# crowsonkb/style_transfer

Hardware: AMD Instinct MI355X
Metric: tile-iterations/sec, VGG-19 2048px/1024-tile (fwd+bwd, Gram/content losses, regularizers, Adam step) (higher is better)
Workload: dtype f32 (fp16x2-split MFMA, fp32 accumulate)

## Files before the change

### include/stx.h

```cpp
#ifndef STX_H_
#define STX_H_

#include <stddef.h>
#include <stdint.h>

#ifdef __cplusplus
extern "C" {
#endif

typedef struct stx_engine stx_engine;

typedef enum stx_status {
    STX_OK = 0,
    STX_ERR_ARG = -1,
    STX_ERR_HIP = -2,
    STX_ERR_STATE = -3,
    STX_ERR_UNSUPPORTED = -4,
    STX_ERR_NOMEM = -5
} stx_status;

typedef enum stx_mem { STX_HOST = 0, STX_DEVICE = 1 } stx_mem;

typedef enum stx_layer_type {
    STX_LAYER_INPUT = 0, STX_LAYER_CONV = 1, STX_LAYER_RELU = 2, STX_LAYER_POOL = 3
// ... 14 lines not shown
} stx_layer_desc;

const char *stx_version(void);
const char *stx_last_error(void);
int stx_reread_env(void);
int stx_device_count(int *count);
int stx_device_name(int device, char *buf, size_t buf_len);

int stx_engine_create(int device, const stx_layer_desc *layers, int n_layers, stx_engine **out);
int stx_engine_create_shared(stx_engine *primary, stx_engine **out);
void stx_engine_destroy(stx_engine *e);
int stx_set_conv_weights(stx_engine *e, const char *conv_layer, const float *weights,
                         const float *bias, int mem);
int stx_sync(stx_engine *e);
int stx_fence(stx_engine *e, unsigned long long *ticket);
int stx_fence_wait(stx_engine *e, unsigned long long ticket);
int stx_engine_wait(stx_engine *e, stx_engine *other);
typedef enum stx_query {
    STX_Q_SHARED_ENGINES = 0,
    STX_Q_TARGET_UPLOADS = 1,
    STX_Q_TARGET_BYTES = 2,
    STX_Q_WEIGHT_BYTES = 3,
    STX_Q_TILE_EVALS = 4,
    STX_Q_PEERS_WITHOUT_ACCESS = 5
} stx_query;
int stx_engine_query(stx_engine *e, int what, double *value);
int stx_engine_device(stx_engine *e, int *device);
int stx_engine_stream(stx_engine *e, void **hip_stream);

int stx_malloc(stx_engine *e, size_t bytes, void **dev_ptr);
int stx_free(stx_engine *e, void *dev_ptr);
int stx_memset_async(stx_engine *e, void *dev_ptr, int value, size_t bytes);
int stx_memcpy_async(stx_engine *e, void *dst, int dst_mem, const void *src, int src_mem,
                     size_t bytes);

typedef struct stx_content_target {
    int content_index;
    const char *layer;
    int channels, height, width;
    const float *features;
    int mem;
} stx_content_target;

typedef struct stx_style_target {
    int style_index;
    const char *layer;
    int channels;
// ... 232 lines not shown
```

### style_transfer_amd/build.py

```python

import concurrent.futures
import os
import subprocess
import sys

CSRC = os.path.join(os.path.dirname(os.path.abspath(__file__)), 'csrc')
REPO = os.path.dirname(os.path.dirname(os.path.abspath(__file__)))
INCLUDE = os.path.join(REPO, 'include')
LIB = os.path.join(CSRC, 'libstx.so')
HIPCC = os.environ.get('HIPCC', '/opt/rocm/bin/hipcc')
ARCH = 'gfx950'

SOURCES = {
    'conv_mfma.hip': [],
    'conv_wino2.hip': [],
    'conv_first.hip': [],
    'conv_h2.hip': [],
    'gram.hip': [],
    'symm.hip': [],
    'pool.hip': [],
    'reduce.hip': [],
    'content_mask.hip': [],
    'image_ops.hip': ['-ffp-contract=off'],
    'swt.hip': ['-ffp-contract=off'],
    'style_mask.hip': ['-ffp-contract=off'],
    'lap.hip': ['-ffp-contract=off'],
    'stat.hip': ['-ffp-contract=off'],
    'photo.hip': ['-ffp-contract=off'],
    'nnfm.hip': ['-ffp-contract=off'],
    'conv_dispatch.cpp': [],
    'engine.cpp': [],
    'targets.cpp': [],
    'tile_path.cpp': [],
    'tile_terms.cpp': [],
    'image_api.cpp': [],
    'op_hooks.cpp': [],
}
EXTRA = os.environ.get('STX_HIPCC_EXTRA', '').split()
COMMON = EXTRA + ['--offload-arch=' + ARCH, '-O3', '-std=c++17', '-fPIC', '-I' + INCLUDE, '-I' + CSRC,
          '-Wall', '-Wno-unused-function']


def _stale(target, deps):
    if not os.path.exists(target):
        return True
    t = os.path.getmtime(target)
    return any(os.path.getmtime(d) > t for d in deps)


def _compile(src, extra, force):
    obj = os.path.join(CSRC, os.path.splitext(src)[0] + '.o')
    path = os.path.join(CSRC, src)
    deps = [path, os.path.join(CSRC, 'common.h'), os.path.join(CSRC, 'bf16x3.h'),
            os.path.join(CSRC, 'f16x2.h'), os.path.join(CSRC, 'engine.h'), os.path.join(INCLUDE, 'stx.h')]
    if force or _stale(obj, deps):
        cmd = [HIPCC] + COMMON + extra + ['-c', path, '-o', obj]
        proc = subprocess.run(cmd, stdout=subprocess.PIPE, stderr=subprocess.STDOUT, text=True)
        if proc.returncode != 0:
            raise RuntimeError('hipcc failed on %s:\n%s' % (src, proc.stdout))
        if proc.stdout.strip():
            sys.stderr.write(proc.stdout)
    return obj


def build(force=False, verbose=False):
    with concurrent.futures.ThreadPoolExecutor(max_workers=min(16, len(SOURCES))) as ex:
        futs = [ex.submit(_compile, src, extra, force) for src, extra in SOURCES.items()]
        objs = [f.result() for f in futs]
    if force or _stale(LIB, objs):
        cmd = [HIPCC, '--offload-arch=' + ARCH, '-shared', '-fPIC', '-o', LIB] + objs
        proc = subprocess.run(cmd, stdout=subprocess.PIPE, stderr=subprocess.STDOUT, text=True)
        if proc.returncode != 0:
            raise RuntimeError('link failed:\n' + proc.stdout)
    if verbose:
        print('built', LIB)
    return LIB

# ... 4 lines not shown
```

### style_transfer_amd/csrc/common.h

```cpp
#pragma once

#include <hip/hip_runtime.h>

#include <vector>

#include <cstdarg>
#include <cstdio>
#include <functional>
#include <string>

#include "stx.h"

namespace stx {

constexpr float kEps = 1.1920928955078125e-07f;

void set_error(const char *fmt, ...);

const char *sw_env(const char *name);
void sw_reread();

#define STX_HIP(call)                                                                       \
    do {                                                                                    \
        hipError_t err__ = (call);                                                          \
// ... 98 lines not shown
    const float *mask;
    float *partials;
    int K, M, H, W;
    int ksize;
    int relu;
    int epilogue;
    ConvInject inject;
    unsigned char *pool_codes = nullptr;
    unsigned char *in_codes = nullptr;
    const unsigned char *mask_codes = nullptr;
    unsigned char *out_codes = nullptr;
    bool wants_codes = false;
    bool skip_y = false;
    float *pool_out = nullptr;
    int pool_mode = 0;
    float *splitk_ws = nullptr;
    size_t splitk_ws_floats = 0;
    long long *clock_out = nullptr;
    const unsigned *x_amax = nullptr;
    unsigned *y_amax = nullptr;
    const unsigned char *pin_codes = nullptr;
    int pin_mode = 0;
    bool pin_mask = false;
#ifdef STX_EXPERIMENT_BF3
    const void *x_split = nullptr;
#endif
};

enum class ConvFamily { Direct, Wino2, H2 };

struct ConvConfig {
    ConvFamily family;
    int id;
    int bm;
    int kc;
    int pr, pc;
    int threads;
    size_t lds_bytes;
};

ConvConfig conv_pick_config(int ksize, int K, int M, int H, int W);
ConvConfig conv_config_by_id(int id);
bool direct_takes_inject(const ConvConfig &cfg);
int conv_num_workgroups(const ConvConfig &cfg, int M, int H, int W);
size_t conv_packed_floats(const ConvConfig &cfg, int K, int M, int ksize);
int conv_pack_weights(hipStream_t s, const float *w_caffe, int Mo, int Ko, int ksize,
// ... 50 lines not shown
                      int K, int H, int W, int relu, float *gram_partials, unsigned *y_amax = nullptr);

ConvConfig wino2_config(int geometry = 0);
int wino2_pick_geometry(int H, int W);
size_t wino2_packed_floats(int K, int M);
int wino2_pack_weights(hipStream_t s, const float *w_caffe, int Mo, int Ko, int transpose_flip,
                       float *packed);
int wino2_launch(hipStream_t s, const ConvConfig &cfg, const ConvProblem &p, int ksplit);
bool wino2_fuses_pool(const ConvProblem &p);
bool wino2_uses_relu_codes(const ConvProblem &p, int ksplit);
bool wino2_writes_out_codes(const ConvConfig &cfg, const ConvProblem &p);
int wino2_splitk_factor(const ConvConfig &cfg, const ConvProblem &p);
struct Wino2Tail { int items, slices; };
Wino2Tail wino2_tail_split(const ConvConfig &cfg, const ConvProblem &p);
int wino2_max_slices(const ConvConfig &cfg, const ConvProblem &p);

constexpr int kAmaxSlots = 64;
ConvConfig h2_config(int mb, int pb = 1);
ConvConfig h2_pick_config(const ConvProblem &p);
bool h2_usable(const ConvProblem &p);
size_t h2_packed_floats(int K, int M);
int h2_pack_weights(hipStream_t s, const float *w_caffe, int Mo, int Ko, int transpose_flip, float *packed);
int h2_launch(hipStream_t s, const ConvConfig &cfg, const ConvProblem &p, int ksplit);
int h2_splitk_factor(const ConvConfig &cfg, const ConvProblem &p);
bool h2_fuses_pool(const ConvProblem &p);
bool h2_takes_pooled_input(const ConvConfig &cfg, const ConvProblem &p);
int absmax_launch(hipStream_t s, const float *x, size_t n, unsigned *slots);

size_t conv_small_packed_floats(int K);
int conv_small_pack(hipStream_t s, const float *w_caffe, int Mo, int Ko, int transpose_flip,
                    float *packed);
int conv_small_launch(hipStream_t s, const float *x, const float *packed, float *y,
                      const float *mask, int K, int M, int H, int W);

bool conv_h2_enabled();
struct ConvTuner { int device; hipStream_t stream; hipEvent_t ev0, ev1; std::function<int(const ConvConfig &, const float **)> bank; };
int conv_choose(const ConvProblem &p, bool winograd, const ConvTuner *tuner, ConvConfig *out);
struct ConvBank { int key; size_t floats; std::function<int(hipStream_t, const float *w_caffe, float *packed)> pack; };
ConvBank conv_bank(const ConvConfig &cfg, int dir, int Mo, int Ko, int ksize);
ConvBank conv_small_bank(int Mo, int Ko);
int conv_dispatch(hipStream_t s, const ConvConfig &cfg, const ConvProblem &p, double *flop_algorithmic,
                  double *flop_issued);
int conv_splitk_factor(const ConvConfig &cfg, const ConvProblem &p);
size_t conv_splitk_floats(const ConvConfig &cfg, const ConvProblem &p);
bool conv_takes_clock(const ConvConfig &cfg);
bool conv_fuses_pool(const ConvConfig &cfg, const ConvProblem &p);
// ... 220 lines not shown
```

### style_transfer_amd/csrc/conv_h2.hip

```cpp

#include <algorithm>
#include <cstdlib>
#include <type_traits>

#include "common.h"
#include "f16x2.h"

#ifndef STX_H2_SKIP
#define STX_H2_SKIP 0
#endif

namespace stx {

namespace {

typedef _Float16 f16x8 __attribute__((ext_vector_type(8)));
typedef float f32x16 __attribute__((ext_vector_type(16)));
typedef float f32x4 __attribute__((ext_vector_type(4)));
typedef float f32x2 __attribute__((ext_vector_type(2)));
typedef unsigned int u32x4 __attribute__((ext_vector_type(4)));
typedef unsigned int u32x3 __attribute__((ext_vector_type(3)));
typedef unsigned int u32x2v __attribute__((__vector_size__(2 * sizeof(unsigned int))));

constexpr int KC = 16;
// ... 21 lines not shown
template <int I, int N, typename F>
__device__ __forceinline__ void static_for(F &&f) {
    if constexpr (I < N) {
        f(std::integral_constant<int, I>{});
        static_for<I + 1, N>(f);
    }
}

__device__ __forceinline__ void lds_barrier() {
    asm volatile("s_waitcnt lgkmcnt(0)\n\ts_barrier" ::: "memory");
}


}

#ifdef STX_H2_TIMING
__device__ long long g_h2_timing[8][8];
__device__ long long g_h2_epi[8][8];
#define STX_H2_STAMP(i) if (pass == 0) t_epi[i] = clock64()
#else
#define STX_H2_STAMP(i)
#endif

template <int EPI, int MB, int PB, int PIN>
__global__ __launch_bounds__(NT) void conv_h2_kernel(WinoArgs a) {
    using G = Geo<PB>;
    [[maybe_unused]] constexpr int PR = G::PR, RT = G::RT, V_PIECE = G::V_PIECE, V_BYTES = G::V_BYTES, NU = G::NU, FULL = G::FULL;
    constexpr size_t kLdsBytes = G::kLds;
    constexpr int NJ = 4 * PB;
    extern __shared__ __attribute__((aligned(16))) char ldsb[];
#ifdef STX_H2_TIMING
    const long long t_start = clock64(), w_start = wall_clock64();
#endif
    constexpr int BM = 64 * MB;

    const int tid = threadIdx.x, lane = tid & 63;
    const int wave = sgpr(tid >> 6);
    const int xi = wave & 3, wh = wave >> 2;
    const int l31 = lane & 31, half = lane >> 5;

    const int m_tiles = a.m_tiles, a_tiles_x = a.tiles_x, a_tiles_y = a.tiles_y, a_H = a.H, a_W = a.W;
    const int a_n_chunks = a.n_chunks, a_ksplit = a.ksplit, a_item_base = a.item_base, a_x_bytes = a.x_bytes,
              a_w_bytes = a.w_bytes;
    const float *const a_x = a.x, *const a_w = a.w;
    asm volatile("" ::"s"(m_tiles), "s"(a_tiles_x), "s"(a_tiles_y), "s"(a_H), "s"(a_W), "s"(a_n_chunks), "s"(a_ksplit),
                 "s"(a_item_base), "s"(a_x_bytes), "s"(a_w_bytes), "s"(a_x), "s"(a_w));
    const int nb = gridDim.x, xcd = blockIdx.x & 7, slot_x = blockIdx.x >> 3;
    const int q8 = nb >> 3, r8 = nb & 7;
// ... 253 lines not shown
#pragma unroll
        for (int q = 0; q < 2; ++q) bq[slot][q] = *reinterpret_cast<const f16x8 *>(vb + q * V_PIECE);
    };

#ifdef STX_H2_TIMING
    const long long t_p0 = clock64();
#endif
    static_for<0, NU>([&](auto n_c) __attribute__((always_inline)) { x_load(decltype(n_c)::value, c_begin); });
    if (LEAN) {
        a_load(0, 0, c_begin);
    } else {
#pragma unroll
        for (int ky = 0; ky < 3; ++ky) a_load(ky, ky, c_begin);
    }
    __builtin_amdgcn_sched_barrier(0);
    read_scales();
#pragma unroll
    for (int b = 0; b < MB; ++b)
#pragma unroll
        for (int j = 0; j < NJ; ++j) asm volatile("" : "+v"(acc[b][j]));
    float s_scale = 0.f, c_scale = 0.f;
    if (EPI == kEpiDgradInject) {
        const float n = (float)((size_t)a.M * HW);
        if (a.inj.sgrad) s_scale = a.inj.s_coef * (1.0f / (a.inj.s_abs_sum[0] / n + kEps));
        if (a.inj.content) c_scale = a.inj.c_coef * (1.0f / (a.inj.c_sums[1] / n + kEps));
    }
    const int hh = wave & 1, mrow = (wave >> 1) & 1, rqp = wave >> 2;
    const bool weven = (a.W & 1) == 0;
    const int xx0 = x0 + 2 * (l31 & 15);
    const unsigned plane_bytes = (unsigned)a.M * HW4;
    const __amdgpu_buffer_rsrc_t ry = __builtin_amdgcn_make_buffer_rsrc(
        a.y + (EPI == kEpiPartial ? (size_t)kslice * a.M * HW : 0), 0, (int)plane_bytes, 0x00020000);
    const __amdgpu_buffer_rsrc_t rmask = __builtin_amdgcn_make_buffer_rsrc(
        const_cast<float *>(a.mask), 0, a.mask ? (int)plane_bytes : 0, 0x00020000);
    const __amdgpu_buffer_rsrc_t rsg = __builtin_amdgcn_make_buffer_rsrc(
        const_cast<float *>(a.inj.sgrad), 0, a.inj.sgrad ? (int)plane_bytes : 0, 0x00020000);
    const __amdgpu_buffer_rsrc_t rft = __builtin_amdgcn_make_buffer_rsrc(
        const_cast<float *>(a.inj.feat), 0, a.inj.feat ? (int)plane_bytes : 0, 0x00020000);
    const __amdgpu_buffer_rsrc_t rbias = __builtin_amdgcn_make_buffer_rsrc(
        const_cast<float *>(a.bias), 0, a.bias ? a.M * 4 : 0, 0x00020000);
    const int ph = (a.H + 1) >> 1, pw = (a.W + 1) >> 1;
    const __amdgpu_buffer_rsrc_t rpool = __builtin_amdgcn_make_buffer_rsrc(
        a.pool_out, 0, a.pool_out ? a.M * ph * pw * 4 : 0, 0x00020000);
    const __amdgpu_buffer_rsrc_t rcodes = __builtin_amdgcn_make_buffer_rsrc(
        a.pool_codes, 0, a.pool_codes ? a.M * ph * pw : 0, 0x00020000);
    const int cph = (a.H + 1) >> 1, cpw = (a.W + 1) >> 1;
    const __amdgpu_buffer_rsrc_t rmc = __builtin_amdgcn_make_buffer_rsrc(
        const_cast<unsigned char *>(a.mask_codes), 0, a.mask_codes ? a.M * cph * cpw : 0, 0x00020000);
// ... 29 lines not shown
        if (decltype(even_c)::value)
            return __builtin_bit_cast(f32x2, __builtin_amdgcn_raw_buffer_load_b64(rs, lr.vo[y][0], so, 0));
        f32x2 v;
        v.x = __builtin_bit_cast(float, __builtin_amdgcn_raw_buffer_load_b32(rs, lr.vo[y][0], so, 0));
        v.y = __builtin_bit_cast(float, __builtin_amdgcn_raw_buffer_load_b32(rs, lr.vo[y][1], so, 0));
        return v;
    };
    auto st2 = [&](const __amdgpu_buffer_rsrc_t &rs, const LaneRows &lr, int y, unsigned so, f32x2 v, auto even_c)
                   __attribute__((always_inline)) {
        if (STX_H2_SKIP & 8) {
            if (v.x == 1.2345e-30f) __builtin_amdgcn_raw_buffer_store_b32(0u, rs, lr.vo[y][0], so, 0);
            return;
        }
        if (decltype(even_c)::value) {
            __builtin_amdgcn_raw_buffer_store_b64(__builtin_bit_cast(u32x2v, v), rs, lr.vo[y][0], so, 0);
        } else {
            const float v0 = v.x, v1 = v.y;
            __builtin_amdgcn_raw_buffer_store_b32(__builtin_bit_cast(unsigned, v0), rs, lr.vo[y][0], so, 0);
            __builtin_amdgcn_raw_buffer_store_b32(__builtin_bit_cast(unsigned, v1), rs, lr.vo[y][1], so, 0);
        }
    };
    int ccol[2] = {0, 0};
    auto content_columns = [&](const LaneRows &lr) __attribute__((always_inline)) {
        if (EPI == kEpiDgradInject && content) {
#pragma unroll
            for (int e = 0; e < 2; ++e) {
                const bool ok = lr.yy < a.H && xx0 < a.W;
                const int x = ok ? (xx0 + e < a.W ? xx0 + e : xx0) : (e && 1 < a.W ? 1 : 0);
                int r = (cw_ox + x) % cw_cw;
                ccol[e] = r < 0 ? r + cw_cw : r;
            }
        }
    };
    if (HOIST) content_columns(rows0);
#ifdef STX_H2_TIMING
    __builtin_amdgcn_sched_barrier(0);
    const long long t_p1 = clock64();
    asm volatile("s_waitcnt vmcnt(0)" ::: "memory");
    const long long t_p2 = clock64();
#endif
    static_for<0, NU>([&](auto n_c) __attribute__((always_inline)) {
        constexpr int n = decltype(n_c)::value;
        stage_all(n, 0);
        if (c_begin + 1 < c_end) x_load(n, c_begin + 1);
    });
#ifdef STX_H2_TIMING
    __builtin_amdgcn_sched_barrier(0);
// ... 83 lines not shown
    if (mark) {
        const long long dc = clock64() - mark_c, dw = wall_clock64() - mark_w;
        if (tid == 0) {
            a.clock_out[0] = dw >= 100 ? dc : 0;
            a.clock_out[1] = dw >= 100 ? dw : 0;
        }
    }
#ifdef STX_H2_TIMING
    const long long t_end = clock64(), w_end = wall_clock64();
#endif

    float amax = 0.f;
    f32x4 *ex = reinterpret_cast<f32x4 *>(ldsb);

#ifdef STX_H2_TIMING
    long long t_epi[4] = {0, 0, 0, 0};
#endif
    auto epilogue_pass = [&](auto pass_c, auto even_c) __attribute__((always_inline)) {
        constexpr int pass = decltype(pass_c)::value;
        constexpr int mbi = pass % MB, pbi = pass / MB;
        const LaneRows lr = pbi == 0 && HOIST ? rows0 : lane_rows(pbi);
        if (!HOIST && pass == 0) content_columns(lr);
        int crow[2] = {0, 0};
        if (EPI == kEpiDgradInject && content) {
#pragma unroll
            for (int y = 0; y < 2; ++y) {
                const bool ok = lr.yy + y < a.H && xx0 < a.W;
                int q = (cw_oy + (ok ? lr.yy + y : 0)) % cw_ch;
                crow[y] = (q < 0 ? q + cw_ch : q) * cw_cw;
            }
        }
        const int cblk = m0 + (hh * MB + mbi) * 32;
        auto chan = [&](int n) __attribute__((always_inline)) {
            const int c0 = cblk + (n & 3) + 8 * (2 * rqp + (n >> 2));
            return sgpr(c0 < M_ ? c0 : M_);
        };
        float bs[8];
        f32x2 mk[16], sg[16];
        unsigned mkb[8];
#pragma unroll
        for (int n = 0; n < 8; ++n) {
            const int c = chan(n);
            const unsigned so = (unsigned)c * HW4;
            if (EPI == kEpiForward) {
                bs[n] = a.bias ? __builtin_bit_cast(float, __builtin_amdgcn_raw_buffer_load_b32(
                                                               rbias, (unsigned)half * 16u, (unsigned)c * 4u, 0))
                               : 0.f;
            } else if (EPI != kEpiPartial) {
                if (a.mask_codes) mkb[n] = __builtin_amdgcn_raw_buffer_load_b8(rmc, lr.vmc, (unsigned)(c * cph * cpw), 0);
#pragma unroll
                for (int y = 0; y < 2; ++y) {
                    if (!a.mask_codes && a.mask && !(STX_H2_SKIP & 16)) mk[2 * n + y] = ld2(rmask, lr, y, so, even_c);
                    if (EPI == kEpiDgradInject && a.inj.sgrad) sg[2 * n + y] = ld2(rsg, lr, y, so, even_c);
                }
            }
        }
        STX_H2_STAMP(0);
        __syncthreads();
        STX_H2_STAMP(1);
#pragma unroll
        for (int j = 0; j < 4; ++j)
#pragma unroll
            for (int rq = 0; rq < 4; ++rq)
                ex[(((xi * 2 + wh) * 4 + j) * 4 + rq) * 64 + lane] =
                    f32x4{acc[mbi][4 * pbi + j][4 * rq], acc[mbi][4 * pbi + j][4 * rq + 1],
                          acc[mbi][4 * pbi + j][4 * rq + 2], acc[mbi][4 * pbi + j][4 * rq + 3]};
        __syncthreads();
        STX_H2_STAMP(2);
#pragma unroll
        for (int rqi = 0; rqi < 2; ++rqi) {
            const int rq = 2 * rqp + rqi;
            f32x4 o[2][2];
#pragma unroll
            for (int s = 0; s < 2; ++s) {
                f32x4 p[4];
#pragma unroll
// ... 1 lines not shown
                o[s][0] = (p[0] + p[1] + p[2]) * out_scale * out_scale2;
                o[s][1] = (p[1] - p[2] - p[3]) * out_scale * out_scale2;
            }
#pragma unroll
            for (int e = 0; e < 4; ++e) {
                const int n = 4 * rqi + e;
                const int c = chan(n);
                const unsigned so = (unsigned)c * HW4;
                f32x2 v[2];
#pragma unroll
                for (int y = 0; y < 2; ++y) v[y] = f32x2{o[y][0][e], o[y][1][e]};
                if (EPI == kEpiForward) {
                    if (a.bias) {
#pragma unroll
                        for (int y = 0; y < 2; ++y) v[y].x += bs[n], v[y].y += bs[n];
                    }
                    if (a.relu) {
#pragma unroll
                        for (int y = 0; y < 2; ++y) v[y].x = fmaxf(v[y].x, 0.f), v[y].y = fmaxf(v[y].y, 0.f);
                    }
                } else if (EPI != kEpiPartial) {
#pragma unroll
                    for (int y = 0; y < 2; ++y) {
                        if (a.mask_codes) {
                            const unsigned nib = mkb[n] >> (2 * y);
                            v[y].x = (nib & 1u) ? v[y].x : 0.f;
                            v[y].y = (nib & 2u) ? v[y].y : 0.f;
                        } else if (a.mask && !(STX_H2_SKIP & 16)) {
                            v[y].x = mk[2 * n + y].x > 0.f ? v[y].x : 0.f;
                            v[y].y = mk[2 * n + y].y > 0.f ? v[y].y : 0.f;
                        }
                        if (EPI == kEpiDgradInject) {
                            if (content) {
                                const f32x2 ft = ld2(rft, lr, y, so, even_c);
                                const int mm = c + 4 * half;
                                const int cm = mm < a.M ? mm : 0;
                                const float *cp = content + (size_t)cm * cw_ch * cw_cw + crow[y];
                                v[y].x += c_scale * (ft.x - cp[ccol[0]]);
                                v[y].y += c_scale * (ft.y - cp[ccol[1]]);
                            }
                            if (a.inj.sgrad) {
                                v[y].x += s_scale * sg[2 * n + y].x;
                                v[y].y += s_scale * sg[2 * n + y].y;
                            }
                        }
                    }
                }
#pragma unroll
                for (int y = 0; y < 2; ++y) {
                    if (EPI != kEpiForward || !a.skip_y) st2(ry, lr, y, so, v[y], even_c);
                    if (EPI != kEpiPartial)
                        amax = fmaxf(amax, fmaxf(lr.vo[y][0] != kOob ? fabsf(v[y].x) : 0.f,
                                                 lr.vo[y][1] != kOob ? fabsf(v[y].y) : 0.f));
                }
                if (EPI == kEpiForward && a.out_codes) {
                    const unsigned nib = (lr.vo[0][0] != kOob && v[0].x > 0.f ? 1u : 0u) |
                                         (lr.vo[0][1] != kOob && v[0].y > 0.f ? 2u : 0u) |
                                         (lr.vo[1][0] != kOob && v[1].x > 0.f ? 4u : 0u) |
                                         (lr.vo[1][1] != kOob && v[1].y > 0.f ? 8u : 0u);
                    __builtin_amdgcn_raw_buffer_store_b8((unsigned char)nib, roc, lr.vmc, (unsigned)(c * cph * cpw), 0);
                }
                if (EPI == kEpiForward && a.pool_out) {
                    const bool hy = lr.yy + 1 < a.H, hx = decltype(even_c)::value || xx0 + 1 < a.W;
                    float pr;
// ... 27 lines not shown
#pragma unroll
        for (int d = 32; d >= 1; d >>= 1) amax = fmaxf(amax, __shfl_xor(amax, d));
        float *wmax = reinterpret_cast<float *>(ldsb + kLdsBytes - 64);
        if (lane == 0) wmax[wave] = amax;
        __syncthreads();
        if (tid == 0) {
#pragma unroll
            for (int w = 1; w < 8; ++w) amax = fmaxf(amax, wmax[w]);
            atomicMax(a.y_amax + (blockIdx.x & (kAmaxSlots - 1)), __builtin_bit_cast(unsigned, amax));
        }
    }
#ifdef STX_H2_TIMING
    if (blockIdx.x == gridDim.x - 3 && lane == 0) {
        g_h2_timing[wave][0] = t_loop - t_start, g_h2_timing[wave][1] = t_end - t_loop;
        g_h2_timing[wave][2] = clock64() - t_end;
        g_h2_timing[wave][3] = w_loop - w_start, g_h2_timing[wave][4] = w_end - w_loop;
        g_h2_timing[wave][5] = wall_clock64() - w_end;
        for (int i = 0; i < 4; ++i) g_h2_epi[wave][i] = t_epi[i] - t_end;
        g_h2_epi[wave][4] = t_p0 - t_start, g_h2_epi[wave][5] = t_p1 - t_p0, g_h2_epi[wave][6] = t_p2 - t_p1, g_h2_epi[wave][7] = t_p3 - t_p2;
    }
#endif
}

__global__ __launch_bounds__(256) void absmax_kernel(const float *__restrict__ x, size_t n, unsigned *slots) {
    float m = 0.f;
    const size_t head = ((16 - (reinterpret_cast<size_t>(x) & 15)) & 15) >> 2;
    const size_t h = head < n ? head : n;
    const size_t n4 = (n - h) >> 2;
    const f32x4 *x4 = reinterpret_cast<const f32x4 *>(x + h);
    for (size_t i = blockIdx.x * (size_t)256 + threadIdx.x; i < n4; i += (size_t)gridDim.x * 256) {
        const f32x4 v = x4[i];
        m = fmaxf(fmaxf(m, fmaxf(fabsf(v.x), fabsf(v.y))), fmaxf(fabsf(v.z), fabsf(v.w)));
    }
    if (blockIdx.x == 0) {
        if (threadIdx.x < h) m = fmaxf(m, fabsf(x[threadIdx.x]));
        const size_t tail = h + (n4 << 2);
        if (tail + threadIdx.x < n && threadIdx.x < 4) m = fmaxf(m, fabsf(x[tail + threadIdx.x]));
    }
#pragma unroll
    for (int d = 32; d >= 1; d >>= 1) m = fmaxf(m, __shfl_xor(m, d));
    __shared__ float wmax[4];
    if ((threadIdx.x & 63) == 0) wmax[threadIdx.x >> 6] = m;
    __syncthreads();
    if (threadIdx.x == 0)
        atomicMax(slots + (blockIdx.x & (kAmaxSlots - 1)),
                  __builtin_bit_cast(unsigned, fmaxf(fmaxf(wmax[0], wmax[1]), fmaxf(wmax[2], wmax[3]))));
// ... 133 lines not shown
}

ConvConfig h2_pick_config(const ConvProblem &p) {
    int f;
    ConvConfig best = h2_config(1, 1);
    double best_cost = h2_plan(best, p, &f);
    const ConvConfig cand[2] = {h2_config(2, 1), h2_config(1, 2)};
    for (int i = 0; i < 2; ++i) {
        if (i == 0 && p.M % 128 != 0) continue;
        const double c = h2_plan(cand[i], p, &f);
        if (c < best_cost) best_cost = c, best = cand[i];
    }
    return best;
}

bool h2_takes_pooled_input(const ConvConfig &cfg, const ConvProblem &p) {
    return p.epilogue == kEpiDgrad && h2_usable(p) && h2_splitk_factor(cfg, p) == 1;
}

bool h2_fuses_pool(const ConvProblem &p) {
    return p.pool_out && p.epilogue == kEpiForward && (((size_t)p.y | (size_t)p.pool_out) & 7) == 0;
}

template <int EPI, int MB, int PB, int PIN = 0>
static int h2_launch_epi(hipStream_t s, const WinoArgs &args, int n_wg) {
    auto kern = conv_h2_kernel<EPI, MB, PB, PIN>;
    constexpr size_t kLdsBytes = Geo<PB>::kLds;
    hipError_t e = hipFuncSetAttribute(reinterpret_cast<const void *>(kern),
                                       hipFuncAttributeMaxDynamicSharedMemorySize, (int)kLdsBytes);
    if (e != hipSuccess) {
        set_error("hipFuncSetAttribute(lds=%zu): %s", kLdsBytes, hipGetErrorString(e));
        return STX_ERR_HIP;
    }
    kern<<<n_wg, NT, kLdsBytes, s>>>(args);
    STX_CHECK_LAUNCH();
    return STX_OK;
}

#ifdef STX_H2_DEV_SUBSET
template __global__ void conv_h2_kernel<0, 2, 1, 0>(WinoArgs);
template __global__ void conv_h2_kernel<0, 1, 2, 0>(WinoArgs);
template __global__ void conv_h2_kernel<1, 2, 1, 0>(WinoArgs);
template __global__ void conv_h2_kernel<3, 2, 1, 0>(WinoArgs);
template __global__ void conv_h2_kernel<3, 1, 2, 1>(WinoArgs);
#else
int h2_launch(hipStream_t s, const ConvConfig &cfg, const ConvProblem &p, int ksplit) {
    if (!h2_usable(p) || !p.x_amax) {
        set_error("h2_launch: unsupported problem (K %d, epilogue %d, input maximum %s)", p.K, p.epilogue,
                  p.x_amax ? "given" : "missing");
        return STX_ERR_UNSUPPORTED;
    }
    WinoArgs a;
    a.x = p.x;
    a.w = p.w;
    a.y = p.y;
    a.bias = p.bias;
    a.mask = p.mask;
    a.K = p.K;
    a.M = p.M;
    a.H = p.H;
    a.W = p.W;
    a.n_chunks = p.K / KC;
    a.tiles_x = ceil_div(p.W, PC);
    a.tiles_y = ceil_div(p.H, cfg.pr);
    a.m_tiles = ceil_div(p.M, cfg.bm);
    a.ksplit = 1;
    a.w_tile_stride = 0;
    a.relu = p.relu;
// ... 15 lines not shown
    }
    a.w_bytes = (int)(4 * (h2_packed_floats(p.K, p.M) - kHeaderFloats));
    a.clock_out = p.clock_out;
    a.x_amax = p.x_amax;
    a.y_amax = p.y_amax;
    a.mask_codes = p.epilogue == kEpiDgrad ? p.mask_codes : nullptr;
    a.out_codes = p.epilogue == kEpiForward && p.relu ? p.out_codes : nullptr;
    const bool inject = p.epilogue == kEpiDgrad && (p.inject.sgrad || p.inject.content);
    int n_wg = a.m_tiles * a.tiles_x * a.tiles_y;
    const bool split = ksplit > 1 && p.splitk_ws && p.splitk_ws_floats >= (size_t)ksplit * p.M * p.H * p.W;
    if (split) {
        a.ksplit = ksplit;
        a.y = p.splitk_ws;
        a.y_amax = nullptr;
        a.mask_codes = nullptr;
        a.out_codes = nullptr;
        n_wg *= ksplit;
    } else if (h2_fuses_pool(p)) {
        a.pool_out = p.pool_out;
        a.pool_codes = p.pool_codes;
        a.skip_y = p.skip_y && p.pool_codes != nullptr;
    }
    const int epi = split ? kEpiPartial : inject ? kEpiDgradInject : p.epilogue;
#define STX_H2_CASE(E)                                                                   \
    case E:                                                                              \
        STX_TRY(cfg.id == 1   ? (h2_launch_epi<E, 2, 1>(s, a, n_wg))                   \
                : cfg.id == 2 ? (h2_launch_epi<E, 1, 2>(s, a, n_wg))                   \
                                : (h2_launch_epi<E, 1, 1>(s, a, n_wg)));                 \
        break;
#define STX_H2_PIN_CASE(E, P)                                                            \
    case E:                                                                              \
        STX_TRY(cfg.id == 1   ? (h2_launch_epi<E, 2, 1, P>(s, a, n_wg))                \
                : cfg.id == 2 ? (h2_launch_epi<E, 1, 2, P>(s, a, n_wg))                \
                                : (h2_launch_epi<E, 1, 1, P>(s, a, n_wg)));              \
        break;
    if (pin && p.pin_mode == STX_POOL_MAX) {
        switch (epi) {
            STX_H2_PIN_CASE(kEpiDgrad, 1 + STX_POOL_MAX)
            STX_H2_PIN_CASE(kEpiDgradInject, 1 + STX_POOL_MAX)
        }
        return STX_OK;
    }
    if (pin) {
        switch (epi) {
            STX_H2_PIN_CASE(kEpiDgrad, 1 + STX_POOL_AVE)
            STX_H2_PIN_CASE(kEpiDgradInject, 1 + STX_POOL_AVE)
        }
        return STX_OK;
    }
#undef STX_H2_PIN_CASE
    switch (epi) {
        STX_H2_CASE(kEpiForward)
        STX_H2_CASE(kEpiDgrad)
        STX_H2_CASE(kEpiDgradInject)
        STX_H2_CASE(kEpiPartial)
        default:
            set_error("h2_launch: no kernel for epilogue %d", p.epilogue);
            return STX_ERR_UNSUPPORTED;
    }
#undef STX_H2_CASE
    return split ? splitk_reduce_launch(s, p, ksplit) : STX_OK;
}
#endif

}
```

### style_transfer_amd/csrc/engine.cpp

```cpp

#include <algorithm>
#include <atomic>
#include <cstdlib>
#include <cstring>

#include "engine.h"

namespace stx {

static thread_local std::string g_error;

void set_error(const char *fmt, ...) {
    char buf[1024];
    va_list ap;
    va_start(ap, fmt);
    vsnprintf(buf, sizeof buf, fmt, ap);
    va_end(ap);
    g_error = buf;
}

int alloc_scalars(stx_engine *e, size_t n, size_t *index) {
    stx_engine::ScalarArena &a = e->A();
    if (a.used + n > e->scalars_cap) {
        set_error("scalar arena exhausted (%zu + %zu > %zu)", a.used, n, e->scalars_cap);
// ... 478 lines not shown
    STX_TRY(e->set_device());
    STX_HIP(hipStreamWaitEvent(e->stream, ev, 0));
    return STX_OK;
}

int stx_engine_query(stx_engine *e, int what, double *value) {
    if (!e || !value) return STX_ERR_ARG;
    std::lock_guard<std::mutex> lock(e->sh->mutex);
    switch (what) {
        case STX_Q_SHARED_ENGINES: *value = (double)e->sh->members.size(); break;
        case STX_Q_TARGET_UPLOADS: *value = (double)e->sh->target_uploads; break;
        case STX_Q_TARGET_BYTES: *value = e->sh->target_bytes; break;
        case STX_Q_WEIGHT_BYTES: {
            double b = 0;
            for (auto &kv : e->sh->conv) {
                b += (double)kv.second.w.bytes + (double)kv.second.b.bytes;
                for (auto &p : kv.second.packed) b += (double)p.second->bytes;
            }
            *value = b;
            break;
        }
        case STX_Q_TILE_EVALS: *value = (double)e->n_tile_evals; break;
        case STX_Q_PEERS_WITHOUT_ACCESS: *value = (double)peers_without_access(e->device); break;
        default:
            set_error("stx_engine_query: unknown item %d", what);
            return STX_ERR_ARG;
    }
    return STX_OK;
}

int stx_malloc(stx_engine *e, size_t bytes, void **dev_ptr) {
    if (!e || !dev_ptr) return STX_ERR_ARG;
    STX_TRY(e->set_device());
    hipError_t err = hipMalloc(dev_ptr, bytes ? bytes : 4);
    if (err != hipSuccess) {
        set_error("hipMalloc(%zu): %s", bytes, hipGetErrorString(err));
        return STX_ERR_NOMEM;
    }
    return STX_OK;
}

int stx_free(stx_engine *e, void *dev_ptr) {
    if (!e) return STX_ERR_ARG;
    STX_TRY(e->set_device());
    if (dev_ptr) STX_HIP(hipFree(dev_ptr));
    return STX_OK;
// ... 165 lines not shown
```

### style_transfer_amd/csrc/engine.h

```cpp
#pragma once

#include <deque>
#include <map>
#include <memory>
#include <mutex>
#include <string>
#include <vector>

#include "common.h"

namespace stx {

struct DevBuf {
    void *ptr = nullptr;
    size_t bytes = 0;
    int ensure(size_t need) {
        if (need <= bytes) return STX_OK;
        if (ptr) STX_HIP(hipFree(ptr));
        ptr = nullptr;
        bytes = 0;
        const size_t want = (need + 255) & ~(size_t)255;
        hipError_t err = hipMalloc(&ptr, want);
        if (err != hipSuccess) {
            set_error("hipMalloc(%zu bytes) failed: %s", want, hipGetErrorString(err));
// ... 147 lines not shown
    bool first_gram_valid = false;
    DevBuf gram_partials, gram, dsym, dsym_pieces, symm_partials, upload;
    DevBuf term_scratch;
    DevBuf masked_feat, masked_target;
    DevBuf stat_scratch;
    DevBuf nnfm_scratch;
    struct ScalarArena {
        DevBuf scalars;
        float *host = nullptr;
        size_t used = 0;
        DevBuf dscalars;
        double *dhost = nullptr;
        size_t dused = 0;
        std::vector<PendingLoss> pending;
        hipEvent_t fence = nullptr;
        unsigned long long ticket = 0;
    };
    ScalarArena arena[2];
    int cur = 0;
    unsigned long long next_ticket = 1;
    ScalarArena &A() { return arena[cur]; }
    size_t scalars_cap = 0;
    size_t n_tile_evals = 0;
    std::vector<hipEvent_t> fence_events;
    size_t fence_next = 0;
    size_t dscalars_cap = 64;
    DevBuf red_scratch;
    DevBuf color_sums;
    DevBuf swt_scratch;
    struct SwtTable {
        int order, levels, N, ntaps, hl;
        DevBuf taps;
    };
    std::vector<SwtTable> swt_tables;
    DevBuf lap_scratch;

    bool winograd = true;
    bool autotune = true;
    bool pool_codes = true;

    bool profiling = false;
    struct ProfEntry {
        std::string label;
        double flops;
        hipEvent_t start, stop;
        int mark = -1;
// ... 181 lines not shown
```

### style_transfer_amd/csrc/tile_path.cpp

```cpp

#include <algorithm>
#include <cmath>
#include <cstdlib>

#include "engine.h"

namespace stx {

ConvProblem conv_fwd_problem(const float *x, float *y, const float *bias, int Cin, int Cout, int H, int W,
                             int ks, int relu) {
    ConvProblem p{};
    p.x = x;
    p.y = y;
    p.bias = bias;
    p.K = Cin;
    p.M = Cout;
    p.H = H;
    p.W = W;
    p.ksize = ks;
    p.relu = relu;
    p.epilogue = kEpiForward;
    return p;
}

// ... 78 lines not shown
static int choose_conv(stx_engine *e, int li, int dir, const ConvProblem &p, ConvConfig *out) {
    const ConvTuner tuner{e->device, e->stream, e->ev_tune0, e->ev_tune1, [=](const ConvConfig &cfg, const float **w) {
                              return get_packed(e, li, dir, cfg, w);
                          }};
    return conv_choose(p, e->winograd, e->autotune ? &tuner : nullptr, out);
}

int attach_splitk(stx_engine *e, const ConvConfig &cfg, ConvProblem &p) {
    const size_t need = conv_splitk_floats(cfg, p);
    if (!need) return STX_OK;
    STX_TRY(e->splitk.ensure(need * sizeof(float)));
    p.splitk_ws = e->splitk.f();
    p.splitk_ws_floats = e->splitk.bytes / sizeof(float);
    return STX_OK;
}

int launch_conv(stx_engine *e, const ConvConfig &cfg, const ConvProblem &problem) {
    ConvProblem p = problem;
    e->last_mark = -1;
    if (e->clock_marks && conv_takes_clock(cfg) && e->marks_used < kMaxClockMarks) {
        e->last_mark = e->marks_used++;
        p.clock_out = static_cast<long long *>(e->marks_buf.ptr) + 2 * (size_t)e->last_mark;
    }
    return conv_dispatch(e->stream, cfg, p, &e->flop_algorithmic, &e->flop_issued);
}

static int amax_for(stx_engine *e, int blob, bool diff, const std::string &consumer, const unsigned **out) {
    Blob &b = e->blobs[blob];
    int &src = diff ? b.amax_diff : b.amax_data;
    if (src < 0) {
        ProfScope scope(e, std::string("absmax ") + b.name, 0.0);
        STX_TRY(absmax_launch(e->stream, diff ? b.diff.f() : b.data.f(), b.count(), e->amax_slots(blob, diff)));
        src = blob;
    } else if (e->amax_audit) {
        STX_TRY(amax_audit_note(e, e->stream, consumer, b.name, diff, e->amax_slots(src, diff),
                                diff ? b.diff.f() : b.data.f(), b.count()));
    }
    *out = e->amax_slots(src, diff);
    return STX_OK;
}

int amax_audit_note(stx_engine *e, hipStream_t stream, const std::string &consumer, const std::string &blob,
                    bool diff, const unsigned *slots, const float *x, size_t n) {
    if (!e->amax_audit) return STX_OK;
    if (e->audit.size() >= kMaxAmaxAudit) {
        set_error("stx_amax_audit: more than %zu hand-offs since the last stx_amax_audit_read", kMaxAmaxAudit);
        return STX_ERR_STATE;
// ... 414 lines not shown
    TileRun run{e, plan, pl, std::vector<std::vector<Term>>(order.size()), {}};
    while (e->sgrad.size() < order.size()) e->sgrad.emplace_back(new DevBuf);
    for (size_t k = 0; k < order.size(); ++k) STX_TRY(e->sgrad[k]->ensure(plan.sgrad_floats[k] * sizeof(float)));
    STX_TRY(e->term_scratch.ensure(plan.scratch_floats * sizeof(float)));
    STX_TRY(begin_timing(e));
    std::vector<char> observed(e->blobs.size(), 0);
    for (const Tap &tp : order) observed[tp.blob] = 1;
    first_gram_setup(e, plan);
    STX_TRY(forward(e, plan.needed, order[0].blob, plan.interleave ? &run : nullptr, true, observed));
    if (!plan.interleave) {
        for (size_t k = order.size(); k-- > 0;) STX_TRY(queue_tap_terms(run, k));
    }
    if (!run.sum_jobs.empty()) {
        ProfScope scope(e, "sums", 0.0);
        STX_TRY(sum_jobs_launch(e->stream, run.sum_jobs.data(), (int)run.sum_jobs.size()));
    }
    STX_TRY(backward_walk(run));
    STX_TRY(end_timing(e));
    STX_HIP(hipMemcpyAsync(e->A().host, e->A().scalars.ptr, e->A().used * sizeof(float),
                           hipMemcpyDeviceToHost, e->stream));
    return STX_OK;
}

static int sc_grad_eager(stx_engine *e, const TileCall &c, double *loss_out) {
    TilePlan plan;
    STX_TRY(sc_grad_prepare(e, c, plan));
    if (e->A().used + plan.scalars > e->scalars_cap) STX_TRY(do_sync(e));
    if (plan.scalars > e->scalars_cap) {
        set_error("stx_sc_grad_tile: %d taps need more scalar space than the arena holds", c.n_taps);
        return STX_ERR_NOMEM;
    }
    Blob &in = e->blobs[e->layers[0].top_blob];
    if (c.img != in.data.ptr) STX_TRY(copy_in(e, in.data.ptr, c.img, c.img_mem, in.count() * sizeof(float)));
    PendingLoss pl;
    pl.out = loss_out;
    STX_TRY(sc_grad_run(e, plan, pl));
    if (c.grad_out != in.diff.ptr)
        STX_TRY(copy_out(e, c.grad_out, c.grad_mem, in.diff.ptr, in.count() * sizeof(float)));
    e->A().pending.push_back(std::move(pl));
    ++e->n_tile_evals;
    return STX_OK;
}

}

extern "C" {

int stx_features_tile(stx_engine *e, const float *img, int img_mem, int th, int tw,
                      const char *const *layers, int n_layers, float *const *out, int out_mem) {
    if (!e || !img || th <= 0 || tw <= 0 || n_layers <= 0 || !layers || !out) {
        set_error("stx_features_tile: bad arguments");
        return STX_ERR_ARG;
    }
    STX_TRY(e->set_device());
    std::vector<char> needed(e->blobs.size(), 0);
    std::vector<int> want(n_layers);
    for (int i = 0; i < n_layers; ++i) {
        want[i] = e->find_blob(layers[i]);
        if (want[i] < 0 || !out[i]) {
            set_error("stx_features_tile: unknown layer '%s'", layers[i] ? layers[i] : "(null)");
            return STX_ERR_ARG;
        }
        mark_ancestors(e, want[i], needed);
// ... 142 lines not shown
```

### style_transfer_amd/lib.py

```python

import ctypes
import os

_HERE = os.path.dirname(os.path.abspath(__file__))
LIB_PATH = os.environ.get('STX_LIB') or os.path.join(_HERE, 'csrc', 'libstx.so')

HOST, DEVICE = 0, 1
LAYER_INPUT, LAYER_CONV, LAYER_RELU, LAYER_POOL = 0, 1, 2, 3
POOL_MAX, POOL_AVE = 0, 1
(Q_SHARED_ENGINES, Q_TARGET_UPLOADS, Q_TARGET_BYTES, Q_WEIGHT_BYTES, Q_TILE_EVALS,
 Q_PEERS_WITHOUT_ACCESS) = range(6)

c_float_p = ctypes.POINTER(ctypes.c_float)
c_double_p = ctypes.POINTER(ctypes.c_double)
c_int_p = ctypes.POINTER(ctypes.c_int)


class StxError(RuntimeError):

    def __init__(self, func, code, message):
        super().__init__('%s failed with status %d: %s' % (func, code, message))
        self.code = code


class LayerDesc(ctypes.Structure):
    _fields_ = [('name', ctypes.c_char_p), ('type', ctypes.c_int), ('bottom', ctypes.c_char_p),
                ('top', ctypes.c_char_p), ('num_output', ctypes.c_int),
                ('kernel_size', ctypes.c_int), ('pad', ctypes.c_int), ('stride', ctypes.c_int),
                ('pool_mode', ctypes.c_int)]


class ContentTarget(ctypes.Structure):
    _fields_ = [('content_index', ctypes.c_int), ('layer', ctypes.c_char_p),
                ('channels', ctypes.c_int), ('height', ctypes.c_int), ('width', ctypes.c_int),
# ... 192 lines not shown
```

Baseline: 279.4.

## Specialise H2 inject-epilogue kernels and bind tile I/O buffers directly

Adds compile-time VAR specialisations of the H2 conv kernel's dgrad-inject epilogue, covering style-only or content-only injection with either nibble or blob masks. These are built in a separate translation unit and chosen by h2_variant, which drops runtime branches and unused loads from the inner epilogue. Separately, when the input image or gradient buffer is a suitably aligned local device allocation with a single small first-conv reader, the engine temporarily points the input blob at the caller's buffers instead of copying in and out. Both changes add bookkeeping counters and query items, and the direct-I/O path depends on pointer-attribute checks and overlap checks being correct.

```diff
diff --git a/include/stx.h b/include/stx.h
--- a/include/stx.h
+++ b/include/stx.h
@@ -60,7 +60,10 @@
     STX_Q_TARGET_BYTES = 2,
     STX_Q_WEIGHT_BYTES = 3,
     STX_Q_TILE_EVALS = 4,
-    STX_Q_PEERS_WITHOUT_ACCESS = 5
+    STX_Q_PEERS_WITHOUT_ACCESS = 5,
+    STX_Q_TILE_IO_DIRECT = 6,
+    STX_Q_INJECT_SPECIALISED = 7,
+    STX_Q_INJECT_VARIANTS = 8
 } stx_query;
 int stx_engine_query(stx_engine *e, int what, double *value);
 int stx_engine_device(stx_engine *e, int *device);
diff --git a/style_transfer_amd/build.py b/style_transfer_amd/build.py
--- a/style_transfer_amd/build.py
+++ b/style_transfer_amd/build.py
@@ -15,7 +15,8 @@
     'conv_mfma.hip': [],
     'conv_wino2.hip': [],
     'conv_first.hip': [],
-    'conv_h2.hip': [],
+    'conv_h2.hip': ['-DSTX_H2_SPLIT_UNITS'],
+    'conv_h2_inject.hip': [],
     'gram.hip': [],
     'symm.hip': [],
     'pool.hip': [],
@@ -53,6 +54,8 @@
     path = os.path.join(CSRC, src)
     deps = [path, os.path.join(CSRC, 'common.h'), os.path.join(CSRC, 'bf16x3.h'),
             os.path.join(CSRC, 'f16x2.h'), os.path.join(CSRC, 'engine.h'), os.path.join(INCLUDE, 'stx.h')]
+    if src == 'conv_h2_inject.hip':
+        deps.append(os.path.join(CSRC, 'conv_h2.hip'))
     if force or _stale(obj, deps):
         cmd = [HIPCC] + COMMON + extra + ['-c', path, '-o', obj]
         proc = subprocess.run(cmd, stdout=subprocess.PIPE, stderr=subprocess.STDOUT, text=True)
diff --git a/style_transfer_amd/csrc/common.h b/style_transfer_amd/csrc/common.h
--- a/style_transfer_amd/csrc/common.h
+++ b/style_transfer_amd/csrc/common.h
@@ -144,6 +144,7 @@
     const unsigned char *pin_codes = nullptr;
     int pin_mode = 0;
     bool pin_mask = false;
+    int *variant_out = nullptr;
 #ifdef STX_EXPERIMENT_BF3
     const void *x_split = nullptr;
 #endif
@@ -240,6 +241,9 @@
 size_t h2_packed_floats(int K, int M);
 int h2_pack_weights(hipStream_t s, const float *w_caffe, int Mo, int Ko, int transpose_flip, float *packed);
 int h2_launch(hipStream_t s, const ConvConfig &cfg, const ConvProblem &p, int ksplit);
+enum { kH2Style = 1, kH2Content = 2, kH2MaskNibbles = 4, kH2MaskBlob = 8 };
+int h2_variant(const ConvProblem &p, int pin, bool split);
+int h2_launch_variant(hipStream_t s, const WinoArgs &a, int n_wg, int cfg_id, int pin, int var);
 int h2_splitk_factor(const ConvConfig &cfg, const ConvProblem &p);
 bool h2_fuses_pool(const ConvProblem &p);
 bool h2_takes_pooled_input(const ConvConfig &cfg, const ConvProblem &p);
diff --git a/style_transfer_amd/csrc/conv_h2.hip b/style_transfer_amd/csrc/conv_h2.hip
--- a/style_transfer_amd/csrc/conv_h2.hip
+++ b/style_transfer_amd/csrc/conv_h2.hip
@@ -67,8 +67,14 @@
 #define STX_H2_STAMP(i)
 #endif
 
-template <int EPI, int MB, int PB, int PIN>
+template <int EPI, int MB, int PB, int PIN, int VAR = 0>
 __global__ __launch_bounds__(NT) void conv_h2_kernel(WinoArgs a) {
+    static_assert(VAR == 0 || EPI == kEpiDgradInject, "variants are of the injecting epilogue");
+    static_assert(VAR == 0 || (((VAR & 3) == 1 || (VAR & 3) == 2) && ((VAR >> 2) == 1 || (VAR >> 2) == 2)), "h2_variant's codes");
+    const bool inj_style = VAR ? (VAR & 1) != 0 : a.inj.sgrad != nullptr;
+    const bool inj_content = VAR ? (VAR & 2) != 0 : a.inj.content != nullptr;
+    const bool mask_nibbles = VAR ? (VAR >> 2) == 1 : a.mask_codes != nullptr;
+    const bool mask_blob = VAR ? (VAR >> 2) == 2 : !a.mask_codes && a.mask;
     using G = Geo<PB>;
     [[maybe_unused]] constexpr int PR = G::PR, RT = G::RT, V_PIECE = G::V_PIECE, V_BYTES = G::V_BYTES, NU = G::NU, FULL = G::FULL;
     constexpr size_t kLdsBytes = G::kLds;
@@ -368,8 +374,8 @@
     float s_scale = 0.f, c_scale = 0.f;
     if (EPI == kEpiDgradInject) {
         const float n = (float)((size_t)a.M * HW);
-        if (a.inj.sgrad) s_scale = a.inj.s_coef * (1.0f / (a.inj.s_abs_sum[0] / n + kEps));
-        if (a.inj.content) c_scale = a.inj.c_coef * (1.0f / (a.inj.c_sums[1] / n + kEps));
+        if (inj_style) s_scale = a.inj.s_coef * (1.0f / (a.inj.s_abs_sum[0] / n + kEps));
+        if (inj_content) c_scale = a.inj.c_coef * (1.0f / (a.inj.c_sums[1] / n + kEps));
     }
     const int hh = wave & 1, mrow = (wave >> 1) & 1, rqp = wave >> 2;
     const bool weven = (a.W & 1) == 0;
@@ -445,7 +451,7 @@
     };
     int ccol[2] = {0, 0};
     auto content_columns = [&](const LaneRows &lr) __attribute__((always_inline)) {
-        if (EPI == kEpiDgradInject && content) {
+        if (EPI == kEpiDgradInject && inj_content) {
 #pragma unroll
             for (int e = 0; e < 2; ++e) {
                 const bool ok = lr.yy < a.H && xx0 < a.W;
@@ -575,7 +581,7 @@
         const LaneRows lr = pbi == 0 && HOIST ? rows0 : lane_rows(pbi);
         if (!HOIST && pass == 0) content_columns(lr);
         int crow[2] = {0, 0};
-        if (EPI == kEpiDgradInject && content) {
+        if (EPI == kEpiDgradInject && inj_content) {
 #pragma unroll
             for (int y = 0; y < 2; ++y) {
                 const bool ok = lr.yy + y < a.H && xx0 < a.W;
@@ -600,11 +606,11 @@
                                                                rbias, (unsigned)half * 16u, (unsigned)c * 4u, 0))
                                : 0.f;
             } else if (EPI != kEpiPartial) {
-                if (a.mask_codes) mkb[n] = __builtin_amdgcn_raw_buffer_load_b8(rmc, lr.vmc, (unsigned)(c * cph * cpw), 0);
+                if (mask_nibbles) mkb[n] = __builtin_amdgcn_raw_buffer_load_b8(rmc, lr.vmc, (unsigned)(c * cph * cpw), 0);
 #pragma unroll
                 for (int y = 0; y < 2; ++y) {
-                    if (!a.mask_codes && a.mask && !(STX_H2_SKIP & 16)) mk[2 * n + y] = ld2(rmask, lr, y, so, even_c);
-                    if (EPI == kEpiDgradInject && a.inj.sgrad) sg[2 * n + y] = ld2(rsg, lr, y, so, even_c);
+                    if (mask_blob && !(STX_H2_SKIP & 16)) mk[2 * n + y] = ld2(rmask, lr, y, so, even_c);
+                    if (EPI == kEpiDgradInject && inj_style) sg[2 * n + y] = ld2(rsg, lr, y, so, even_c);
                 }
             }
         }
@@ -652,16 +658,16 @@
                 } else if (EPI != kEpiPartial) {
 #pragma unroll
                     for (int y = 0; y < 2; ++y) {
-                        if (a.mask_codes) {
+                        if (mask_nibbles) {
                             const unsigned nib = mkb[n] >> (2 * y);
                             v[y].x = (nib & 1u) ? v[y].x : 0.f;
                             v[y].y = (nib & 2u) ? v[y].y : 0.f;
-                        } else if (a.mask && !(STX_H2_SKIP & 16)) {
+                        } else if (mask_blob && !(STX_H2_SKIP & 16)) {
                             v[y].x = mk[2 * n + y].x > 0.f ? v[y].x : 0.f;
                             v[y].y = mk[2 * n + y].y > 0.f ? v[y].y : 0.f;
                         }
                         if (EPI == kEpiDgradInject) {
-                            if (content) {
+                            if (inj_content) {
                                 const f32x2 ft = ld2(rft, lr, y, so, even_c);
                                 const int mm = c + 4 * half;
                                 const int cm = mm < a.M ? mm : 0;
@@ -669,7 +675,7 @@
                                 v[y].x += c_scale * (ft.x - cp[ccol[0]]);
                                 v[y].y += c_scale * (ft.y - cp[ccol[1]]);
                             }
-                            if (a.inj.sgrad) {
+                            if (inj_style) {
                                 v[y].x += s_scale * sg[2 * n + y].x;
                                 v[y].y += s_scale * sg[2 * n + y].y;
                             }
@@ -743,6 +749,43 @@
 #endif
 }
 
+template <int EPI, int MB, int PB, int PIN = 0, int VAR = 0>
+static int h2_launch_epi(hipStream_t s, const WinoArgs &args, int n_wg) {
+    auto kern = conv_h2_kernel<EPI, MB, PB, PIN, VAR>;
+    constexpr size_t kLdsBytes = Geo<PB>::kLds;
+    hipError_t e = hipFuncSetAttribute(reinterpret_cast<const void *>(kern),
+                                       hipFuncAttributeMaxDynamicSharedMemorySize, (int)kLdsBytes);
+    if (e != hipSuccess) {
+        set_error("hipFuncSetAttribute(lds=%zu): %s", kLdsBytes, hipGetErrorString(e));
+        return STX_ERR_HIP;
+    }
+    kern<<<n_wg, NT, kLdsBytes, s>>>(args);
+    STX_CHECK_LAUNCH();
+    return STX_OK;
+}
+
+#if defined(STX_H2_VARIANTS_ONLY) || !(defined(STX_H2_SPLIT_UNITS) || defined(STX_H2_DEV_SUBSET))
+int h2_launch_variant(hipStream_t s, const WinoArgs &a, int n_wg, int cfg_id, int pin, int var) {
+#define STX_H2_VAR(V, P)                                                                                      \
+    if (var == (V) && pin == (P))                                                                             \
+        return cfg_id == 1   ? h2_launch_epi<kEpiDgradInject, 2, 1, P, V>(s, a, n_wg)                         \
+               : cfg_id == 2 ? h2_launch_epi<kEpiDgradInject, 1, 2, P, V>(s, a, n_wg)                         \
+                             : h2_launch_epi<kEpiDgradInject, 1, 1, P, V>(s, a, n_wg);
+    STX_H2_VAR(kH2Style | kH2MaskNibbles, 0)
+    STX_H2_VAR(kH2Style | kH2MaskBlob, 0)
+    STX_H2_VAR(kH2Content | kH2MaskNibbles, 0)
+    STX_H2_VAR(kH2Content | kH2MaskBlob, 0)
+    STX_H2_VAR(kH2Style | kH2MaskNibbles, 1 + STX_POOL_MAX)
+    STX_H2_VAR(kH2Style | kH2MaskBlob, 1 + STX_POOL_MAX)
+    STX_H2_VAR(kH2Style | kH2MaskNibbles, 1 + STX_POOL_AVE)
+    STX_H2_VAR(kH2Style | kH2MaskBlob, 1 + STX_POOL_AVE)
+#undef STX_H2_VAR
+    set_error("h2_launch_variant: no specialised body %d for a pooled input of kind %d", var, pin);
+    return STX_ERR_UNSUPPORTED;
+}
+#endif
+#ifndef STX_H2_VARIANTS_ONLY
+
 __global__ __launch_bounds__(256) void absmax_kernel(const float *__restrict__ x, size_t n, unsigned *slots) {
     float m = 0.f;
     const size_t head = ((16 - (reinterpret_cast<size_t>(x) & 15)) & 15) >> 2;
@@ -922,28 +965,28 @@
     return p.pool_out && p.epilogue == kEpiForward && (((size_t)p.y | (size_t)p.pool_out) & 7) == 0;
 }
 
-template <int EPI, int MB, int PB, int PIN = 0>
-static int h2_launch_epi(hipStream_t s, const WinoArgs &args, int n_wg) {
-    auto kern = conv_h2_kernel<EPI, MB, PB, PIN>;
-    constexpr size_t kLdsBytes = Geo<PB>::kLds;
-    hipError_t e = hipFuncSetAttribute(reinterpret_cast<const void *>(kern),
-                                       hipFuncAttributeMaxDynamicSharedMemorySize, (int)kLdsBytes);
-    if (e != hipSuccess) {
-        set_error("hipFuncSetAttribute(lds=%zu): %s", kLdsBytes, hipGetErrorString(e));
-        return STX_ERR_HIP;
-    }
-    kern<<<n_wg, NT, kLdsBytes, s>>>(args);
-    STX_CHECK_LAUNCH();
-    return STX_OK;
-}
-
 #ifdef STX_H2_DEV_SUBSET
 template __global__ void conv_h2_kernel<0, 2, 1, 0>(WinoArgs);
 template __global__ void conv_h2_kernel<0, 1, 2, 0>(WinoArgs);
 template __global__ void conv_h2_kernel<1, 2, 1, 0>(WinoArgs);
 template __global__ void conv_h2_kernel<3, 2, 1, 0>(WinoArgs);
 template __global__ void conv_h2_kernel<3, 1, 2, 1>(WinoArgs);
+template __global__ void conv_h2_kernel<3, 2, 1, 0, kH2Style | kH2MaskNibbles>(WinoArgs);
+template __global__ void conv_h2_kernel<3, 2, 1, 0, kH2Content | kH2MaskNibbles>(WinoArgs);
+template __global__ void conv_h2_kernel<3, 1, 2, 1, kH2Style | kH2MaskBlob>(WinoArgs);
+template __global__ void conv_h2_kernel<3, 2, 1, 1, kH2Style | kH2MaskNibbles>(WinoArgs);
 #else
+int h2_variant(const ConvProblem &p, int pin, bool split) {
+    if (split || p.epilogue != kEpiDgrad) return 0;
+    const bool style = p.inject.sgrad != nullptr, content = p.inject.content != nullptr;
+    if (style == content) return 0;
+    if (!p.mask_codes && !p.mask) return 0;
+    if (content && pin) return 0;
+    const char *env = sw_env("STX_H2_INJECT_GENERIC");
+    if (env && atoi(env) != 0) return 0;
+    return (style ? kH2Style : kH2Content) | (p.mask_codes ? kH2MaskNibbles : kH2MaskBlob);
+}
+
 int h2_launch(hipStream_t s, const ConvConfig &cfg, const ConvProblem &p, int ksplit) {
     if (!h2_usable(p) || !p.x_amax) {
         set_error("h2_launch: unsupported problem (K %d, epilogue %d, input maximum %s)", p.K, p.epilogue,
@@ -1005,6 +1048,10 @@
         a.skip_y = p.skip_y && p.pool_codes != nullptr;
     }
     const int epi = split ? kEpiPartial : inject ? kEpiDgradInject : p.epilogue;
+    const int pin_kind = pin ? 1 + p.pin_mode : 0;
+    const int var = h2_variant(p, pin_kind, split);
+    if (p.variant_out) *p.variant_out = var;
+    if (var) return h2_launch_variant(s, a, n_wg, cfg.id, pin_kind, var);
 #define STX_H2_CASE(E)                                                                   \
     case E:                                                                              \
         STX_TRY(cfg.id == 1   ? (h2_launch_epi<E, 2, 1>(s, a, n_wg))                   \
@@ -1045,5 +1092,6 @@
     return split ? splitk_reduce_launch(s, p, ksplit) : STX_OK;
 }
 #endif
-
-}
+#endif
+
+}
diff --git a/style_transfer_amd/csrc/conv_h2_inject.hip b/style_transfer_amd/csrc/conv_h2_inject.hip
--- /dev/null
+++ b/style_transfer_amd/csrc/conv_h2_inject.hip
@@ -0,0 +1,2 @@
+#define STX_H2_VARIANTS_ONLY
+#include "conv_h2.hip"
diff --git a/style_transfer_amd/csrc/engine.cpp b/style_transfer_amd/csrc/engine.cpp
--- a/style_transfer_amd/csrc/engine.cpp
+++ b/style_transfer_amd/csrc/engine.cpp
@@ -524,6 +524,9 @@
         }
         case STX_Q_TILE_EVALS: *value = (double)e->n_tile_evals; break;
         case STX_Q_PEERS_WITHOUT_ACCESS: *value = (double)peers_without_access(e->device); break;
+        case STX_Q_TILE_IO_DIRECT: *value = (double)e->n_tile_io_direct; break;
+        case STX_Q_INJECT_SPECIALISED: *value = (double)e->n_inject_specialised; break;
+        case STX_Q_INJECT_VARIANTS: *value = (double)e->inject_variants; break;
         default:
             set_error("stx_engine_query: unknown item %d", what);
             return STX_ERR_ARG;
diff --git a/style_transfer_amd/csrc/engine.h b/style_transfer_amd/csrc/engine.h
--- a/style_transfer_amd/csrc/engine.h
+++ b/style_transfer_amd/csrc/engine.h
@@ -193,6 +193,9 @@
     ScalarArena &A() { return arena[cur]; }
     size_t scalars_cap = 0;
     size_t n_tile_evals = 0;
+    size_t n_tile_io_direct = 0;
+    size_t n_inject_specialised = 0;
+    unsigned inject_variants = 0;
     std::vector<hipEvent_t> fence_events;
     size_t fence_next = 0;
     size_t dscalars_cap = 64;
diff --git a/style_transfer_amd/csrc/tile_path.cpp b/style_transfer_amd/csrc/tile_path.cpp
--- a/style_transfer_amd/csrc/tile_path.cpp
+++ b/style_transfer_amd/csrc/tile_path.cpp
@@ -124,7 +124,14 @@
         e->last_mark = e->marks_used++;
         p.clock_out = static_cast<long long *>(e->marks_buf.ptr) + 2 * (size_t)e->last_mark;
     }
-    return conv_dispatch(e->stream, cfg, p, &e->flop_algorithmic, &e->flop_issued);
+    int var = 0;
+    p.variant_out = &var;
+    const int rc = conv_dispatch(e->stream, cfg, p, &e->flop_algorithmic, &e->flop_issued);
+    if (var) {
+        ++e->n_inject_specialised;
+        e->inject_variants |= 1u << var;
+    }
+    return rc;
 }
 
 static int amax_for(stx_engine *e, int blob, bool diff, const std::string &consumer, const unsigned **out) {
@@ -585,6 +592,70 @@
     return STX_OK;
 }
 
+static bool local_device_floats(const stx_engine *e, const void *p, int mem) {
+    if (mem == STX_HOST || (reinterpret_cast<uintptr_t>(p) & 3) != 0) return false;
+    hipPointerAttribute_t attr{};
+    if (hipPointerGetAttributes(&attr, p) != hipSuccess) {
+        (void)hipGetLastError();
+        return false;
+    }
+    return attr.type == hipMemoryTypeDevice && attr.device == e->device;
+}
+
+static bool ranges_overlap(const void *a, const void *b, size_t bytes) {
+    const uintptr_t x = reinterpret_cast<uintptr_t>(a), y = reinterpret_cast<uintptr_t>(b);
+    return x < y + bytes && y < x + bytes;
+}
+
+static void tile_io_direct(stx_engine *e, const TileCall &c, const TilePlan &plan, bool *in_direct, bool *out_direct) {
+    const int data_blob = e->layers[0].top_blob;
+    const Blob &in = e->blobs[data_blob];
+    const size_t bytes = in.count() * sizeof(float);
+    *in_direct = *out_direct = false;
+    if (const char *env = sw_env("STX_TILE_IO_DIRECT"))
+        if (atoi(env) == 0) return;
+    if (plan.tap_of[data_blob] >= 0 || in.relu) return;
+    if (ranges_overlap(c.img, c.grad_out, bytes) || ranges_overlap(c.img, in.data.ptr, in.data.bytes) ||
+        ranges_overlap(c.img, in.diff.ptr, in.diff.bytes) || ranges_overlap(c.grad_out, in.data.ptr, in.data.bytes) ||
+        ranges_overlap(c.grad_out, in.diff.ptr, in.diff.bytes))
+        return;
+    std::vector<char> observed(e->blobs.size(), 0);
+    for (const Tap &tp : plan.order) observed[tp.blob] = 1;
+    int readers = 0;
+    bool first_only = true, small_only = true;
+    for (size_t li = 1; li < e->layers.size(); ++li) {
+        const Layer &L = e->layers[li];
+        if (L.type == STX_LAYER_RELU || L.bottom_blob != data_blob || !plan.needed[L.top_blob]) continue;
+        ++readers;
+        if (L.type != STX_LAYER_CONV) {
+            first_only = small_only = false;
+            continue;
+        }
+        const ConvParams &cp = e->sh->conv[li];
+        first_only &= conv_first_usable(cp.cin, cp.cout, cp.ks) &&
+                      !plan_fwd_conv(e, li, plan.needed, plan.order[0].blob, true, observed).pool;
+        small_only &= cp.ks == 3 && cp.cin <= 4;
+    }
+    if (readers != 1) return;
+    *in_direct = first_only && local_device_floats(e, c.img, c.img_mem);
+    *out_direct = small_only && local_device_floats(e, c.grad_out, c.grad_mem);
+}
+
+struct TileIoView {
+    Blob &in;
+    void *const data, *const diff;
+    TileIoView(Blob &blob, const void *img, void *grad) : in(blob), data(blob.data.ptr), diff(blob.diff.ptr) {
+        if (img) in.data.ptr = const_cast<void *>(img);
+        if (grad) in.diff.ptr = grad;
+    }
+    ~TileIoView() {
+        in.data.ptr = data;
+        in.diff.ptr = diff;
+    }
+    TileIoView(const TileIoView &) = delete;
+    TileIoView &operator=(const TileIoView &) = delete;
+};
+
 static int sc_grad_eager(stx_engine *e, const TileCall &c, double *loss_out) {
     TilePlan plan;
     STX_TRY(sc_grad_prepare(e, c, plan));
@@ -594,14 +665,21 @@
         return STX_ERR_NOMEM;
     }
     Blob &in = e->blobs[e->layers[0].top_blob];
-    if (c.img != in.data.ptr) STX_TRY(copy_in(e, in.data.ptr, c.img, c.img_mem, in.count() * sizeof(float)));
+    bool in_direct, out_direct;
+    tile_io_direct(e, c, plan, &in_direct, &out_direct);
+    if (c.img != in.data.ptr && !in_direct)
+        STX_TRY(copy_in(e, in.data.ptr, c.img, c.img_mem, in.count() * sizeof(float)));
     PendingLoss pl;
     pl.out = loss_out;
-    STX_TRY(sc_grad_run(e, plan, pl));
-    if (c.grad_out != in.diff.ptr)
+    {
+        const TileIoView view(in, in_direct ? c.img : nullptr, out_direct ? c.grad_out : nullptr);
+        STX_TRY(sc_grad_run(e, plan, pl));
+    }
+    if (c.grad_out != in.diff.ptr && !out_direct)
         STX_TRY(copy_out(e, c.grad_out, c.grad_mem, in.diff.ptr, in.count() * sizeof(float)));
     e->A().pending.push_back(std::move(pl));
     ++e->n_tile_evals;
+    e->n_tile_io_direct += (in_direct ? 1 : 0) + (out_direct ? 1 : 0);
     return STX_OK;
 }
 
diff --git a/style_transfer_amd/lib.py b/style_transfer_amd/lib.py
--- a/style_transfer_amd/lib.py
+++ b/style_transfer_amd/lib.py
@@ -9,7 +9,7 @@
 LAYER_INPUT, LAYER_CONV, LAYER_RELU, LAYER_POOL = 0, 1, 2, 3
 POOL_MAX, POOL_AVE = 0, 1
 (Q_SHARED_ENGINES, Q_TARGET_UPLOADS, Q_TARGET_BYTES, Q_WEIGHT_BYTES, Q_TILE_EVALS,
- Q_PEERS_WITHOUT_ACCESS) = range(6)
+ Q_PEERS_WITHOUT_ACCESS, Q_TILE_IO_DIRECT, Q_INJECT_SPECIALISED, Q_INJECT_VARIANTS) = range(9)
 
 c_float_p = ctypes.POINTER(ctypes.c_float)
 c_double_p = ctypes.POINTER(ctypes.c_double)
```

New measurement: 283.3 (median of 6 runs). +1.4%, better.
